# ethan-li-coding/AD-Census

Hardware: AMD Instinct MI355X
Metric: stereo pairs/s at 1920x1080 D=128 (ADCensusStereo::Match, images and disparity map resident in HBM) (higher is better)
Workload: dtype f32; 1 GPU; noise 1920x1080 D=128 (BASELINE.json configs[3]); batch=160 distinct pairs (seeds 12345+i), 668 per GPU (cycled), queue=static round-robin partition, in_flight_per_gpu=1, parallelism=replicas x1 (independent pairs), full=False

## Files before the change

### adcensus_amd/csrc/adc_internal.h

```cpp
#pragma once
#include <hip/hip_runtime.h>
#include <stdint.h>
#include <stddef.h>

#include "../../include/adcensus_c_api.h"

#define ADC_WAVE 64

#if !defined(ADC_VOL_NT) || ADC_VOL_NT
#define ADC_VOL_NT_STR " nt"
#define ADC_VOL_STORE(PTR, VAL) __builtin_nontemporal_store((VAL), (PTR))
#else
#define ADC_VOL_NT_STR ""
#define ADC_VOL_STORE(PTR, VAL) (*(PTR) = (VAL))
#endif


#ifdef ADC_FAULT_INJECTION
extern "C" int adc_test_fault_now(void);
#define ADC_HIP(call) (adc_test_fault_now() ? hipErrorOutOfMemory : (call))
#else
#define ADC_HIP(call) (call)
#endif

// ... 47 lines not shown
    int set;
    adc_raw_format fmt;
    uint32_t* rec;
    float *mx, *my;
    uint8_t* valid;
    uint8_t* raw;
    size_t raw_cap;
};

#define ADC_PIN_ARM 64
#define ADC_PIN_MEDIAN 0
#define ADC_PIN_CLOUD 8
#define ADC_PIN_SPECKLE 9
struct adc_handle {
    AdcParams p;
    int device;
    hipStream_t stream;
    hipStream_t heavy;
    hipEvent_t ev_in, ev_heavy_done;
    bool own_stream;

    uint8_t *img_l, *img_r;
    uint8_t *img_l_own, *img_r_own;
    uint8_t *gray_l, *gray_r;
    uint64_t *census_l, *census_r;
    uint8_t* arms;
    uint16_t *sup_h, *sup_v;
    int* armmax;
    uint32_t *rec_h, *rec_v;
    uint32_t *rec2_h, *rec2_v;
    float* agg_sink;
    uint8_t *cdiff_lh, *cdiff_lv, *cdiff_rh, *cdiff_rv;
    uint8_t* so_cls;
    float* so_seam;
    int so_seg_off;
    int so_nseg_last;
    int so_seam_redos;
    float *vol_a, *vol_b;
    float* lut_ad;
    float* lut_census;
    double* ray_sincos;
    float so_P1[3], so_P2[3];
    float *disp_l, *disp_r, *disp_tmp;
    uint8_t* label;
    uint8_t* elig;
    uint8_t* irv_bbox;
    int32_t* vote_list;
    int32_t* vote_evals_arr;
    int32_t* interp_list;
    int32_t* interp_counters;
    int32_t* ray_tab;
    int ray_tab_rows;
    int32_t* ray_lin;
    int itp_pitch, itp_ms;
    uint32_t* cost_rrec;
    uint32_t* cost_lrec;
    int rrec_pitch, rrec_padl;
    int armmax_host[2];
    int armmax_valid;
    int arm_known;
    int arm_redos;
    int agg_dual;
    int agg_dual_last;
    int agg_last_plan;
    int agg_switches;
    int agg_dual_runs;
    int armmax_small[2];
    int agg_gate, agg_gate_thr;
    int redo_partial;
    int match_pending;
    int fuse_cost;
    int agg_first_fused;
    int fuse_wta;
    int fuse_agg_so;
    int so_agg_fused;
    int agg_so_fusions;
    int32_t* pin_nz;
    long long rec_nz_host[2];
    int rec_nz_known;
    int in_redo;
    int agg_sparse_last;
    int agg_sparse_launches;
    int agg_gather_launches;
    int wta_left_done;
    float* med_hand;
    int med_hpitch;
    float* med_sink;
    int med_spec_off;
    int med_spec_last;
    int med_seg_last;
    int med_seg_off;
    int med_spec_fails;
    int force_median_fallback;
    int median_fallbacks;
    int32_t* pin_flags;
    int bgrx_valid;
    uint32_t* bgrx_l;
    uint16_t* st16;
    int st16_pitch;
    float* disp_vote;
    int irv_xcd_mode;
    int irv_grid;
    int irv_budget;
    int irv_used_hist[8];
    unsigned irv_used_pos;
    int irv_chain;
    int irv_pending;
    int irv_overflows;
    float *tail_disp_l, *tail_disp_tmp;
    void* irv_cold;
    unsigned char irv_cold_host[64];
    int irv_cold_valid, irv_cold_flip;
    int32_t* vote_counters;
    uint32_t* irv_px;
    uint8_t* chg_a;
    int chg_pitch;
    uint8_t* edge;
    uint8_t* itp_cells;
    uint8_t* pin_in;
    float* pin_out;
    AdcMatchReq req;
    AdcMapBuf map_buf[ADC_REQ_MAPS];
    uint32_t* out_words;
    void* os_cloud;
    uint32_t os_cloud_cap;
    int32_t sp_max_size;
    float sp_max_diff;
    int32_t* sp_parent;
    float* sp_map;
    AdcRectSide rect[2];
    uint8_t* pin_raw;
    size_t pin_raw_cap;
    int ev_set;
    int ev_has_right, ev_has_mask;
    float ev_occ_thres;
    int ev_cus;
    float* ev_g[2];
    uint8_t* ev_occ;
    uint8_t* ev_raw;
    size_t ev_raw_cap;
    uint64_t* ev_rep;
    uint64_t* ev_pin;
    int ev_pending;
    adc_eval_report ev_echo;
    adc_eval_report ev_report;
    int ev_report_valid;
    float* evs_disp;
    uint8_t* evs_prov;
    float* evs_conf;
    float* evs_err;
    uint8_t* evs_cls;
    int profiling, verbose;
    hipEvent_t ev[ADC_STAGE_COUNT + 1];
    hipEvent_t ev_agg[9];
    float stage_ms[ADC_STAGE_COUNT];
    float agg_pass_ms;
    int agg_launches;
    int agg_passes;
    const char* agg_kernel;
    uint32_t paper;
    uint8_t* arms_r;
    uint32_t* bgrx_r;
    int* armmax_r;
    float* vol_c;
    bool timings_pending;
    int64_t vote_rounds, vote_evals;
};

hipError_t adc_launch_gray_census(adc_handle* h);
hipError_t adc_launch_cost(adc_handle* h, float* vol_out);
hipError_t adc_launch_cost_records(adc_handle* h);
int adc_agg_small_L(const adc_handle* h);
double adc_agg_sparse_density(void);
double adc_agg_gather_density(void);
hipError_t adc_launch_arms(adc_handle* h);
hipError_t adc_launch_arms_left(adc_handle* h);
hipError_t adc_launch_sup_counts(adc_handle* h);
hipError_t adc_launch_arms_rest(adc_handle* h);
hipError_t adc_launch_aggregate_tail(adc_handle* h);
hipError_t adc_launch_records(adc_handle* h);
hipError_t adc_launch_aggregate(adc_handle* h, int iterations);
hipError_t adc_launch_so_classes(adc_handle* h, hipStream_t stream);
size_t adc_so_cls_bytes(int W, int H);
hipError_t adc_launch_scanline(adc_handle* h, int passes);
int adc_so_segments(const adc_handle* h, int* warm_out);
bool adc_so_can_fuse_agg(const adc_handle* h);
size_t adc_so_seam_bytes(int W, int H, int Dp);
hipError_t adc_launch_wta(adc_handle* h);
hipError_t adc_launch_wta_left(adc_handle* h);
hipError_t adc_paper_aggregate(adc_handle* h, int iterations);
hipError_t adc_paper_accumulate(adc_handle* h, float* acc, const float* src, int first, int last);
hipError_t adc_launch_lrcheck(adc_handle* h);
hipError_t adc_launch_confidence(adc_handle* h);
hipError_t adc_launch_provenance(adc_handle* h);
size_t adc_outputs_scratch_bytes(int W, int H);
hipError_t adc_launch_out_measure(adc_handle* h, const float* disp, const uint8_t* img);
hipError_t adc_launch_out_scan(adc_handle* h);
hipError_t adc_launch_out_emit(adc_handle* h, const float* disp, const uint8_t* img);
hipError_t adc_launch_disp16(adc_handle* h, const float* disp, float scale, uint16_t* out);
size_t adc_speckle_scratch_words(int W, int H);
hipError_t adc_launch_speckle_runs(adc_handle* h, const float* src, float max_diff);
hipError_t adc_launch_speckle_merge(adc_handle* h, const float* src, float max_diff);
hipError_t adc_launch_speckle_flatten(adc_handle* h, int32_t* labels);
hipError_t adc_launch_speckle_apply(adc_handle* h, const float* src, float* dst, uint8_t* prov, int max_size);
hipError_t adc_launch_rect_model_maps(adc_handle* h, int side, const adc_camera_model* m);
hipError_t adc_launch_rect_pack(adc_handle* h, int side);
hipError_t adc_launch_rect_remap(adc_handle* h, int side, const uint8_t* raw, uint8_t* bgr_out);
hipError_t adc_launch_rect_convert(adc_handle* h, int side, const uint8_t* raw, uint8_t* bgr_out);
static inline int adc_pix_code(int format) { return format & 0xff; }
static inline bool adc_pix_is16(int format) { const int c = format & 0xff; return c == ADC_PIX_GRAY16 || (c >= ADC_PIX_BAYER_RGGB16 && c <= ADC_PIX_BAYER_BGGR16); }
static inline int adc_pix_shift(int format) { const int b = (format >> 8) & 0xff; return adc_pix_is16(format) ? (b ? b : 16) - 8 : 0; }
size_t adc_eval_report_words(void);
hipError_t adc_launch_eval_gt(adc_handle* h, int side, int format, int pitch, float scale);
hipError_t adc_launch_eval_occ(adc_handle* h, int mode, float occ_thres);
hipError_t adc_launch_eval_measure(adc_handle* h, const float* disp, const uint8_t* prov, const float* conf, const float* thresholds, float* err, uint8_t* cls);
size_t adc_itp_cell_bytes(int W, int H, int ms);
#define ADC_MEDB_MAX_SEG 12
size_t adc_median_hand_rows(int H);
int adc_irv_probe_xcd_mode(int device);
int adc_irv_grid(size_t pixels);
size_t adc_irv_waves(int grid);
size_t adc_irv_px_words(int W, int H);
size_t adc_irv_list_entries(int W, int H, int D, int grid);
hipError_t adc_run_region_voting(adc_handle* h);
hipError_t adc_voting_finish(adc_handle* h, int* continued);
hipError_t adc_launch_interpolation(adc_handle* h);
hipError_t adc_launch_discontinuity(adc_handle* h);
hipError_t adc_launch_median(adc_handle* h);
hipError_t adc_median_fallback(adc_handle* h);
hipError_t adc_launch_pad_volume(adc_handle* h, const float* src_HWD, float* dst_HWDp);
hipError_t adc_launch_unpad_volume(adc_handle* h, const float* src_HWDp, float* dst_HWD);
```

### adcensus_amd/csrc/capi.hip

```cpp
#include "adc_internal.h"
#include "adc_device_fn.h"

#include <math.h>
#include <stdio.h>
#include <stdlib.h>
#include <string.h>
#include <string>
#include <vector>
#include <new>
#include <mutex>
#include <atomic>

static thread_local std::string g_last_error;

#ifdef ADC_FAULT_INJECTION
static std::atomic<long> g_fi_calls{0};
static std::atomic<long> g_fi_fail_at{[] { const char* e = getenv("ADC_TEST_FAIL_AT"); return e ? atol(e) : 0L; }()};
extern "C" int adc_test_fault_now(void) { const long n = ++g_fi_calls; return n == g_fi_fail_at.load(); }
extern "C" void adc_test_fail_at(long n) { g_fi_calls = 0; g_fi_fail_at = n; }
extern "C" long adc_test_hip_calls(void) { return g_fi_calls.load(); }
#endif

struct HostRange { const char* base; size_t bytes; };
static std::mutex g_host_mu;
// ... 1709 lines not shown
            if (e == hipSuccess && h->pin_nz) e = hipMemcpyAsync(h->pin_nz, h->armmax + ADC_NZ_BASE, 2 * ADC_NZ_SHARDS * ADC_NZ_STRIDE * sizeof(int32_t), hipMemcpyDeviceToHost, h->heavy);
            if (e == hipSuccess && h->pin_nz) e = hipStreamSynchronize(h->heavy);
            if (e == hipSuccess && h->pin_nz) {
                for (int c = 0; c < 2; c++) {
                    h->rec_nz_host[c] = 0;
                    for (int s = 0; s < ADC_NZ_SHARDS; s++) h->rec_nz_host[c] += h->pin_nz[(c * ADC_NZ_SHARDS + s) * ADC_NZ_STRIDE];
                }
                h->rec_nz_known = 1;
            }
            arg -= 200;
        }
        if (e == hipSuccess && arg >= 100) {
            if (h->paper & ADC_PAPER_RIGHT_ARMS) e = adc_launch_cost(h, h->vol_a);
            else { e = adc_launch_cost_records(h); h->fuse_cost = 1; }
            arg -= 100;
        }
        if (e == hipSuccess) e = adc_launch_aggregate(h, arg > 0 ? arg : 4);
        h->fuse_cost = 0;
        h->armmax_valid = 0;
        break;
    case ADC_RUN_SCANLINE:
        h->fuse_wta = arg >= 100 ? 1 : 0;
        h->wta_left_done = 0;
        e = adc_launch_scanline(h, arg >= 100 ? arg - 100 : arg);
        h->fuse_wta = 0;
        break;
    case ADC_RUN_WTA: e = adc_launch_wta(h); break;
    case ADC_RUN_LRCHECK: e = adc_launch_lrcheck(h); break;
    case ADC_RUN_REGION_VOTING:
        if (arg < 0) { h->irv_budget = -arg; return 0; }
        if (arg > 0) h->irv_budget = arg;
        e = adc_launch_sup_counts(h);
        if (e == hipSuccess) e = adc_run_region_voting(h);
        if (e == hipSuccess) e = hipStreamSynchronize(h->stream);
        if (e == hipSuccess) { int cont = 0; e = adc_voting_finish(h, &cont); }
        break;
    case ADC_RUN_INTERPOLATION: e = adc_launch_interpolation(h); break;
    case ADC_RUN_DISCONTINUITY: e = adc_launch_discontinuity(h); break;
    case ADC_RUN_MEDIAN:
        if (arg == 100) { h->force_median_fallback = 1; return 0; }
        if (arg == 101) { h->force_median_fallback = 2; return 0; }
        e = adc_launch_median(h);
        break;
    default: return 1;
    }
    if (e != hipSuccess) { set_error("adc_debug_run launch", e); return 2; }
    e = hipStreamSynchronize(h->heavy);
    if (e == hipSuccess) e = hipStreamSynchronize(h->stream);
    if (e != hipSuccess) { set_error("adc_debug_run sync", e); return 2; }
    if (stage == ADC_RUN_SCANLINE && h->so_nseg_last > 1) {
        int fails = 0;
        if (hipMemcpy(&fails, h->armmax + 2, sizeof(int), hipMemcpyDeviceToHost) != hipSuccess) { set_error("adc_debug_run: seam flag", hipGetLastError()); return 2; }
        if (fails != 0) {
            h->so_seg_off = 64;
            g_last_error = "adc_debug_run(ADC_RUN_SCANLINE): a speculative row segment failed its seam check; rerun with ADC_SO_SEG=1";
            return 3;
        }
    }
    if (stage == ADC_RUN_MEDIAN && h->pin_flags && h->pin_flags[ADC_PIN_MEDIAN] != 0) {
        e = adc_median_fallback(h);
        h->pin_flags[ADC_PIN_MEDIAN] = 0;
        h->median_fallbacks++;
        if (e != hipSuccess) { set_error("adc_debug_run: median fallback", e); return 2; }
    }
    return 0;
}

int64_t adc_debug_counter(adc_handle* h, int which)
{
    if (!h) return -1;
    switch (which) {
    case 0: return h->median_fallbacks;
    case 1: return h->irv_overflows;
    case 2: return h->arm_redos;
    case 9: return h->agg_switches;
    case 10: return h->agg_dual_runs;
    case 11: return h->redo_partial;
    case 12: return h->agg_dual;
    case 13: return h->agg_so_fusions;
    case 16: return h->agg_sparse_launches;
    case 17: return (int64_t)(adc_agg_sparse_density() * 1e6 + 0.5);
    case 20: return h->agg_gather_launches;
    case 21: return (int64_t)(adc_agg_gather_density() * 1e6 + 0.5);
    case 18: return h->rec_nz_known ? h->rec_nz_host[0] : -1;
    case 19: return h->rec_nz_known ? h->rec_nz_host[1] : -1;
    case 14: return h->irv_xcd_mode;
    case 15: return h->med_seg_last;
    case 3: return h->irv_budget;
    case 7: return h->med_spec_fails;
    case 8: return h->med_spec_last;
    case 4: return h->so_seam_redos;
    case 5: return h->so_nseg_last;
    case 6: {
        int v = -1;
        return hipMemcpy(&v, h->armmax + 2, sizeof(int), hipMemcpyDeviceToHost) == hipSuccess ? v : -1;
    }
    default: return -1;
    }
}

int adc_debug_voting_stats(adc_handle* h, int64_t* rounds, int64_t* evaluations)
{
    if (!h) return 1;
    if (rounds) *rounds = h->vote_rounds;
    if (evaluations) *evaluations = h->vote_evals;
    return 0;
}

}
```

### adcensus_amd/csrc/k_aggregate.hip

```cpp
#include "adc_internal.h"
#include "adc_device_fn.h"
#include <mutex>
#include "k_aggregate_rr.h"
#include "k_aggregate_rr2.h"
#include "k_agg_gather.h"

#define AGG_PF 8
#ifndef ADC_K4_TAILLOOP
#define ADC_K4_TAILLOOP 0
#endif
#ifndef ADC_K4_DIAG
#define ADC_K4_DIAG 0
#endif

__device__ __forceinline__ float agg_run(float acc, const float* q, int cnt)
{
    while (cnt >= 8) {
        const float t0 = q[0], t1 = q[64], t2 = q[128], t3 = q[192], t4 = q[256], t5 = q[320], t6 = q[384], t7 = q[448];
        acc += t0; acc += t1; acc += t2; acc += t3; acc += t4; acc += t5; acc += t6; acc += t7;
        q += 512;
        cnt -= 8;
    }
    switch (cnt) {
    case 7: { const float t0 = q[0], t1 = q[64], t2 = q[128], t3 = q[192], t4 = q[256], t5 = q[320], t6 = q[384];
// ... 566 lines not shown

int adc_agg_small_L(const adc_handle* h)
{
    static const int small_L_env = env_int("ADC_AGG_SMALL_L", 8);
    const int L = adc_imax(0, adc_imin(h->p.opt.cross_L1, 255));
    return adc_imin(small_L_env, L);
}

static int pick_nseg(long long nlines, int N, int L, int slots)
{
    int best = 1;
    long long best_cost = -1;
    for (int ns = 1; ns <= 16; ns++) {
        const int seg = (N + ns - 1) / ns;
        if (ns > 1 && seg < 2 * L) break;
        const long long rounds = (nlines * ns + slots - 1) / slots;
        const long long cost = rounds * (seg + (ns > 1 ? 2 * L : 0));
        if (best_cost < 0 || cost < best_cost) { best_cost = cost; best = ns; }
    }
    return best;
}

static int pick_chunk(long long nlines, int N, int L, int slots)
{
    const long long total = nlines * N;
    long long best_cost = -1;
    int best = N;
    auto consider = [&](long long c) {
        if (c < 1) c = 1;
        if (c < N && c < 4 * (long long)L) return;
        if (c > total) c = total;
        const long long waves = (total + c - 1) / c;
        const long long rounds = (waves + slots - 1) / slots;
        const bool aligned = c >= N ? (c % N == 0) : (N % c == 0);
        const long long pieces = aligned ? (c >= N ? c / N : 1) : (c >= N ? c / N + 2 : 2);
        const long long halo = (c < N || !aligned) ? 2LL * L : 0;
        const long long cost = rounds * (c + halo + 60 * pieces);
        if (best_cost < 0 || cost < best_cost) { best_cost = cost; best = (int)c; }
    };
    for (int k = 1; k <= 16; k++) consider((N + k - 1) / k);
    for (int k = 1; k <= 3; k++) consider((total + (long long)slots * k - 1) / ((long long)slots * k));
    return best;
}

static int agg_assumed_depth(const adc_handle* h, bool vert)
{
    const int assume_margin = env_int("ADC_AGG_ASSUME_MARGIN", 1);
    const int Lknown = adc_imax(1, h->armmax_host[vert ? 1 : 0]) + (h->armmax_valid == 2 ? assume_margin : 0);
    return adc_imin(adc_agg_small_L(h), Lknown);
}

static bool agg_small_vpl2(const adc_handle* h, bool pair)
{
    static const int vpl2_env = env_int("ADC_AGG_VPL2", 1);
    return (vpl2_env == 1 || (vpl2_env == 2 && pair)) && h->p.Dp % 128 == 0;
}

#define AGG_SPARSE_MAX_DENSITY 0.105
double adc_agg_sparse_density(void)
{
    const char* e = getenv("ADC_AGG_SPARSE_DENSITY");
    return e ? atof(e) : AGG_SPARSE_MAX_DENSITY;
}
static bool agg_sparse_wanted(const adc_handle* h, bool vert, bool pair)
{
    const char* e = getenv("ADC_AGG_SPARSE");
    if (e && atoi(e) == 0) return false;
    if (h->agg_gate || h->in_redo || !(h->armmax_valid == 1 || h->armmax_valid == 2) || !h->rec_nz_known) return false;
    if (!agg_small_vpl2(h, pair)) return false;
    return (double)h->rec_nz_host[vert ? 1 : 0] <= adc_agg_sparse_density() * (double)h->p.W * (double)h->p.H;
}

#define AGG_GATHER_MAX_DENSITY AGG_SPARSE_MAX_DENSITY
double adc_agg_gather_density(void)
{
    const char* e = getenv("ADC_AGG_GATHER_DENSITY");
    return e ? atof(e) : AGG_GATHER_MAX_DENSITY;
}
static bool agg_gather_wanted(const adc_handle* h, bool vert)
{
    const char* e = getenv("ADC_AGG_GATHER");
    if (e && atoi(e) == 0) return false;
    return (double)h->rec_nz_host[vert ? 1 : 0] <= adc_agg_gather_density() * (double)h->p.W * (double)h->p.H;
}

template <bool VERT, bool DIVIDE, bool COSTIN = false, bool PAIR = false>
static hipError_t launch_pass(adc_handle* h, const float* src, float* dst, int which = 0, bool sparse = false)
{
    const bool gather = sparse && agg_gather_wanted(h, VERT);
    const AdcParams& p = h->p;
    const int L = adc_imax(0, adc_imin(p.opt.cross_L1, 255));
    const int N = VERT ? p.H : p.W;
    const int small_L = adc_agg_small_L(h);
    if (sparse && (COSTIN || which != 1 || !agg_small_vpl2(h, PAIR))) return hipErrorInvalidValue;
    for (int variant = 0; variant < 2; variant++) {
        if (variant == 1 && (small_L <= 0 || small_L >= L)) break;
        if ((which == 1 && variant == 0 && small_L > 0 && small_L < L) || (which == 2 && variant == 1)) continue;
        const int Lv = variant ? ((which == 1 && h->armmax_valid) ? agg_assumed_depth(h, VERT) : small_L) : L;
        static const bool regring_env = env_int("ADC_AGG_REGRING", 1) != 0;
        const bool regring = variant == 0 && regring_env && Lv >= 1 && 2 * Lv + 1 <= AGG_RING_REGS;
        static const bool rr2_env = env_int("ADC_AGG_RR2", 1) != 0;
        const bool rr2 = regring && rr2_env && !PAIR && p.Dp % 128 == 0 && 2 * Lv + 1 <= RR2_SLOTS;
        const int vpl = rr2 ? 2 : ((variant == 1 && !COSTIN && agg_small_vpl2(h, PAIR)) ? 2 : 1);
        const long long nlines = (long long)(VERT ? p.W : p.H) * (p.Dp / (64 * vpl));
        const size_t ring_bytes = regring ? 0 : (size_t)(2 * Lv + 1) * 64 * sizeof(float) * vpl;
        const size_t ldsv = ring_bytes + (COSTIN ? (768 + 64) * sizeof(float) : 0) + ((PAIR && !regring) ? ring_bytes + (2 * Lv + 1) * 4 + 64 : 0);
        const int waves_per_cu = regring ? ((PAIR || rr2) ? 8 : 16) : adc_imax(1, adc_imin(32, (int)((160 * 1024) / ((ldsv + 511) / 512 * 512))));
        int nseg = env_int(VERT ? "ADC_AGG_VSEG" : "ADC_AGG_HSEG", 0);
        if (nseg < 1) nseg = pick_nseg(nlines, N, PAIR ? 2 * Lv : Lv, 256 * waves_per_cu);
        int seg_len = (N + nseg - 1) / nseg;
        if (seg_len < 1) seg_len = 1;
        nseg = (N + seg_len - 1) / seg_len;
        const long long waves = nlines * nseg;
        const int per_xcd = (int)((waves + 7) / 8);
        const bool both = which == 0 && small_L > 0 && small_L < L;
        const bool verify = variant == 1 && which == 1 && h->armmax_valid == 2;
        int sv = both ? variant : (verify ? 2 : -1), sl = both ? small_L : (verify ? Lv : 0x7fffffff);
        if (h->agg_gate) { sv = h->agg_gate; sl = h->agg_gate_thr; }
        AggCostIn ci;
        ci.rrec = reinterpret_cast<const uint4*>(h->cost_rrec);
        ci.lrec = reinterpret_cast<const uint4*>(h->cost_lrec);
        ci.lut_ad = h->lut_ad;
        ci.lut_census = h->lut_census;
        ci.rpitch = h->rrec_pitch; ci.padl = h->rrec_padl; ci.dmin = p.dmin; ci.D = p.D;
        if (!COSTIN)
            h->agg_kernel = rr2 ? "k_agg_rr2 (register ring of VGPR pairs, 2 disparities per lane, one pass per launch)"
                          : regring ? (PAIR ? "k_agg_regring_pair (two register rings, dividing pass + next first pass per launch)"
                                            : "k_agg_regring (register ring, 1 disparity per lane, one pass per launch)")
                          : (variant && gather) ? (PAIR ? "k_agg_gather<.., PAIR> + k_agg_apply (SPARSE launch, gather form: dividing pass + next first pass, only changed pixels computed)"
                                                        : "k_agg_gather + k_agg_apply (SPARSE launch, gather form: one pass per launch, only changed pixels computed)")
                          : (variant && sparse) ? (PAIR ? "k_agg_march<.., PAIR, SPARSE> + k_agg_apply (LDS small rings: dividing pass + next first pass per launch, only changed pixels stored)"
                                                        : "k_agg_march<.., SMALL, SPARSE> + k_agg_apply (LDS small ring, one pass per launch, only changed pixels stored)")
                          : variant ? (PAIR ? "k_agg_march<.., PAIR> (LDS small rings: dividing pass + next first pass per launch)"
                                            : "k_agg_march<.., SMALL> (LDS small ring, one pass per launch)")
                                    : "k_agg_march (LDS full ring, one pass per launch)";
        if (rr2) {
            int chunk_len = env_int(VERT ? "ADC_AGG_VCHUNK" : "ADC_AGG_HCHUNK", 0);
            if (chunk_len < 1) chunk_len = pick_chunk(nlines, N, Lv, 256 * waves_per_cu);
            const long long total = nlines * N;
            const int nwaves = (int)((total + chunk_len - 1) / chunk_len);
            const int pxc = (nwaves + 7) / 8;
            if constexpr (COSTIN)
                hipLaunchKernelGGL(k_agg_rr2_cost, dim3((unsigned)pxc * 8), dim3(64), ldsv, h->heavy, dst,
                                   reinterpret_cast<const uint2*>(h->rec2_h), p.W, p.H, p.Dp, Lv, chunk_len, nwaves, pxc, h->armmax, sv, sl, ci);
            else if constexpr (!PAIR)
                hipLaunchKernelGGL((k_agg_rr2<VERT, DIVIDE>), dim3((unsigned)pxc * 8), dim3(64), 0, h->heavy, src, dst,
                                   reinterpret_cast<const uint2*>(VERT ? h->rec2_v : h->rec2_h), p.W, p.H, p.Dp, Lv, chunk_len, nwaves,
                                   pxc, h->armmax, sv, sl);
        } else if (regring) {
            if constexpr (COSTIN)
                hipLaunchKernelGGL(k_agg_regring_cost, dim3((unsigned)per_xcd * 8), dim3(64), ldsv, h->heavy, src, dst,
                                   VERT ? h->rec_v : h->rec_h, p.W, p.H, p.Dp, Lv, seg_len, nseg, per_xcd, h->armmax, sv, sl, ci);
            else if constexpr (PAIR)
                hipLaunchKernelGGL((k_agg_regring_pair<VERT>), dim3((unsigned)per_xcd * 8), dim3(64), 0, h->heavy, src, dst,
                                   reinterpret_cast<const uint2*>(VERT ? h->rec2_v : h->rec2_h), p.W, p.H, p.Dp, Lv, seg_len, nseg,
                                   per_xcd, h->armmax, sv, sl, h->agg_sink);
            else
                hipLaunchKernelGGL((k_agg_regring<VERT, DIVIDE>), dim3((unsigned)per_xcd * 8), dim3(64), 0, h->heavy, src, dst,
                                   reinterpret_cast<const uint2*>(VERT ? h->rec2_v : h->rec2_h), p.W, p.H, p.Dp, Lv, seg_len, nseg,
                                   per_xcd, h->armmax, sv, sl, h->agg_sink);
        } else if (variant && vpl == 2) {
            if constexpr (!COSTIN) {
                if (sparse) {
                    const long long P = (long long)p.W * p.H;
                    if (gather) {
                        hipLaunchKernelGGL((k_agg_gather<VERT, DIVIDE, PAIR>), dim3((unsigned)((P + 255) / 256)), dim3(256), 0, h->heavy, src, dst,
                                           VERT ? h->rec_v : h->rec_h, p.W, p.H, p.Dp, h->armmax, sv, sl);
                        h->agg_gather_launches++;
                    } else
                        hipLaunchKernelGGL((k_agg_march<VERT, DIVIDE, true, false, PAIR, 2, true>), dim3((unsigned)per_xcd * 8), dim3(64), ldsv, h->heavy, src, dst,
                                           VERT ? h->rec_v : h->rec_h, p.W, p.H, p.Dp, Lv, seg_len, nseg, per_xcd, h->armmax, sv, sl, ci);
                    hipLaunchKernelGGL((k_agg_apply<VERT>), dim3((unsigned)((P + 255) / 256)), dim3(256), 0, h->heavy, dst, const_cast<float*>(src),
                                       VERT ? h->rec_v : h->rec_h, p.W, p.H, p.Dp, (DIVIDE || PAIR) ? 1 : 0, h->armmax, sv, sl);
                    h->agg_sparse_launches++;
                    h->agg_sparse_last = 1;
                } else
                    hipLaunchKernelGGL((k_agg_march<VERT, DIVIDE, true, false, PAIR, 2>), dim3((unsigned)per_xcd * 8), dim3(64), ldsv, h->heavy, src, dst,
                                       VERT ? h->rec_v : h->rec_h, p.W, p.H, p.Dp, Lv, seg_len, nseg, per_xcd, h->armmax, sv, sl, ci);
            }
        } else if (variant)
            hipLaunchKernelGGL((k_agg_march<VERT, DIVIDE, true, COSTIN, PAIR>), dim3((unsigned)per_xcd * 8), dim3(64), ldsv, h->heavy, src, dst,
                               VERT ? h->rec_v : h->rec_h, p.W, p.H, p.Dp, Lv, seg_len, nseg, per_xcd, h->armmax, sv, sl, ci);
        else
            hipLaunchKernelGGL((k_agg_march<VERT, DIVIDE, false, COSTIN, PAIR>), dim3((unsigned)per_xcd * 8), dim3(64), ldsv, h->heavy, src, dst,
                               VERT ? h->rec_v : h->rec_h, p.W, p.H, p.Dp, Lv, seg_len, nseg, per_xcd, h->armmax, sv, sl, ci);
    }
    return hipGetLastError();
}

struct AggSeq { int launches, passes; float* result; bool first_fused; };
static hipError_t agg_sequence(adc_handle* h, int iterations, bool dry, bool first_into_cur, bool marks, AggSeq* out)
{
    static const bool pair_env = env_int("ADC_AGG_PAIR", 1) != 0;
    static const int pair_full = env_int("ADC_AGG_PAIR_FULL", 0);
    static const bool regring_on = env_int("ADC_AGG_REGRING", 1) != 0;
    hipError_t e = hipSuccess;
    const int Lfull = adc_imax(0, adc_imin(h->p.opt.cross_L1, 255));
    const bool regring_fits = regring_on && Lfull >= 1 && 2 * Lfull + 1 <= AGG_RING_REGS;
    const bool lds_fits = (size_t)(2 * Lfull + 1) * 64 * sizeof(float) + (768 + 64) * sizeof(float) <= 150 * 1024;
    const bool marching = true;
    const bool prof = marks && !dry && h->profiling;
    const int small_L = adc_agg_small_L(h);
    const bool small_ok = small_L > 0 && small_L < Lfull;
    int which_h = 0, which_v = 0;
    if (h->armmax_valid == 3 && marching) {
        which_h = which_v = 2;
    } else if (h->armmax_valid && marching) {
        which_h = (small_ok && h->armmax_host[0] <= small_L) ? 1 : 2;
        which_v = (small_ok && h->armmax_host[1] <= small_L) ? 1 : 2;
    }
    float* cur = h->vol_a;
    float* oth = h->vol_b;
    bool horizontal_first = true;
    int launch = 0;
    int passes = 0;
    bool second_done = false;
    bool first_fused = false;
    for (int k = 0; k < iterations && e == hipSuccess; k++) {
        const bool hf = horizontal_first;
        if (!second_done) {
            if (prof && launch < 2) hipEventRecord(h->ev_agg[launch], h->heavy);
            bool swap = true;
            if (hf) {
                const bool fused = k == 0 && h->fuse_cost && lds_fits;
                if (k == 0) first_fused = fused;
                if (fused) {
                    swap = !first_into_cur;
                    if (!dry) e = launch_pass<false, false, true>(h, cur, swap ? oth : cur, which_h);
                } else {
                    const bool sp = which_h == 1 && agg_sparse_wanted(h, false, false);
                    if (!dry) e = launch_pass<false, false>(h, cur, oth, which_h, sp);
                    swap = !sp;
                }
            } else {
                const bool sp = which_v == 1 && agg_sparse_wanted(h, true, false);
                if (!dry) e = launch_pass<true, false>(h, cur, oth, which_v, sp);
                swap = !sp;
            }
            if (swap) { float* t = cur; cur = oth; oth = t; }
            launch++;
            passes++;
        }
        second_done = false;
        if (e != hipSuccess) break;
        if (prof && launch < 2) hipEventRecord(h->ev_agg[launch], h->heavy);
        const int wsec = hf ? which_v : which_h;
        if (!hf && k + 1 == iterations && iterations == 4 && h->fuse_agg_so && !h->agg_gate && marching && which_h == 1 &&
            (h->armmax_valid == 1 || h->armmax_valid == 2) && agg_assumed_depth(h, false) <= 4 && adc_so_can_fuse_agg(h)) {
            if (!dry) { h->so_agg_fused = 1; h->agg_so_fusions++; }
            break;
        }
        const bool pair = pair_env && marching && k + 1 < iterations &&
                          (wsec == 1 || (wsec == 2 && (pair_full >= 2 || (pair_full == 1 && regring_fits))));
        const bool sparse = wsec == 1 && agg_sparse_wanted(h, hf, pair);
        if (!dry) {
            if (hf) {
                if (pair) e = launch_pass<true, true, false, true>(h, cur, oth, wsec, sparse);
                else e = launch_pass<true, true>(h, cur, oth, which_v, sparse);
            } else {
                if (pair) e = launch_pass<false, true, false, true>(h, cur, oth, wsec, sparse);
                else e = launch_pass<false, true>(h, cur, oth, which_h, sparse);
            }
// ... 91 lines not shown
```

### adcensus_amd/csrc/k_cost.hip

```cpp
#include "adc_internal.h"
#include "adc_device_fn.h"

#define CT_W 32
#define CT_H 8
#define CT_LW (CT_W + 6)
#define CT_LH (CT_H + 8)

__global__ __launch_bounds__(CT_W* CT_H) void k_gray_census(const uint8_t* __restrict__ img_l,
                                                             const uint8_t* __restrict__ img_r,
                                                             uint8_t* __restrict__ gray_l, uint8_t* __restrict__ gray_r,
                                                             uint64_t* __restrict__ census_l,
                                                             uint64_t* __restrict__ census_r, int W, int H, int census5)
{
    __shared__ uint8_t tile[CT_LH][CT_LW + 2];
    const uint8_t* img = blockIdx.z == 0 ? img_l : img_r;
    uint8_t* gray = blockIdx.z == 0 ? gray_l : gray_r;
    uint64_t* census = blockIdx.z == 0 ? census_l : census_r;
    const int x0 = blockIdx.x * CT_W, y0 = blockIdx.y * CT_H;
    const int tid = threadIdx.y * CT_W + threadIdx.x;
    for (int i = tid; i < CT_LH * CT_LW; i += CT_W * CT_H) {
        const int ly = i / CT_LW, lx = i % CT_LW;
        const int gx = x0 + lx - 3, gy = y0 + ly - 4;
        uint8_t g = 0;
        if (gx >= 0 && gx < W && gy >= 0 && gy < H) {
            const uint8_t* p = img + ((size_t)gy * W + gx) * 3;
            g = adc_gray(p[0], p[1], p[2]);
        }
        tile[ly][lx] = g;
    }
    __syncthreads();
    const int x = x0 + threadIdx.x, y = y0 + threadIdx.y;
    if (x >= W || y >= H) return;
    const int lx = threadIdx.x + 3, ly = threadIdx.y + 4;
    const uint8_t c = tile[ly][lx];
    gray[(size_t)y * W + x] = c;
    uint64_t v = 0;
    if (census5) {
        if (W > 5 && H > 5 && y >= 2 && y < H - 2 && x >= 2 && x < W - 2) {
#pragma unroll
            for (int r = -2; r <= 2; r++)
#pragma unroll
                for (int cc = -2; cc <= 2; cc++) {
                    v <<= 1;
                    v += (tile[ly + r][lx + cc] < c) ? 1u : 0u;
                }
        }
    } else if (W > 9 && H > 7 && y >= 4 && y < H - 4 && x >= 3 && x < W - 3) {
#pragma unroll
        for (int r = -4; r <= 4; r++)
#pragma unroll
            for (int cc = -3; cc <= 3; cc++) {
                v <<= 1;
                v += (tile[ly + r][lx + cc] < c) ? 1u : 0u;
            }
    }
    census[(size_t)y * W + x] = v;
}

hipError_t adc_launch_gray_census(adc_handle* h)
{
    const AdcParams& p = h->p;
    dim3 grid((p.W + CT_W - 1) / CT_W, (p.H + CT_H - 1) / CT_H, 2), block(CT_W, CT_H, 1);
    hipLaunchKernelGGL(k_gray_census, grid, block, 0, h->heavy, h->img_l, h->img_r, h->gray_l, h->gray_r, h->census_l,
                       h->census_r, p.W, p.H, (h->paper & ADC_PAPER_CENSUS5X5) ? 1 : 0);
    return hipGetLastError();
}

#define COST_TX 32
#define COST_MAXSEG (COST_TX + ADC_MAX_DISP_RANGE)

template <int VPL>
__global__ __launch_bounds__(256) void k_cost(const uint8_t* __restrict__ img_l, const uint8_t* __restrict__ img_r,
                                              const uint64_t* __restrict__ census_l,
                                              const uint64_t* __restrict__ census_r, const float* __restrict__ lut_ad,
                                              const float* __restrict__ lut_census, float* __restrict__ vol, int W,
                                              int H, int dmin, int D)
{
    constexpr int Dp = 64 * VPL;
    __shared__ float sA[768];
    __shared__ float sC[64];
    __shared__ uint32_t sBgr[COST_MAXSEG];
    __shared__ uint64_t sCen[COST_MAXSEG];

    const int y = blockIdx.y;
// ... 25 lines not shown
        const int bl = pl[0], gl = pl[1], rl = pl[2];
        const uint64_t cl = census_l[(size_t)y * W + x];
        float out[VPL];
#pragma unroll
        for (int k = 0; k < VPL; k++) {
            const int di = lane * VPL + k;
            float c = 0.0f;
            if (di < D) {
                const int xr = x - (di + dmin);
                const uint32_t pr = sBgr[xr - xr_lo];
                if (pr == 0xFFFFFFFFu) {
                    c = 1.0f;
                } else {
                    const int ad = adc_iabs(bl - (int)(pr & 255u)) + adc_iabs(gl - (int)((pr >> 8) & 255u)) +
                                   adc_iabs(rl - (int)((pr >> 16) & 255u));
                    const int hm = __popcll(cl ^ sCen[xr - xr_lo]);
                    c = sA[ad] - sC[hm];
                }
            }
            out[k] = c;
        }
        float* dst = vol + ((size_t)y * W + x) * Dp + lane * VPL;
        if constexpr (VPL == 1) dst[0] = out[0];
        else if constexpr (VPL == 2) *reinterpret_cast<float2*>(dst) = make_float2(out[0], out[1]);
        else {
#pragma unroll
            for (int q = 0; q < VPL; q += 4) *reinterpret_cast<float4*>(dst + q) = make_float4(out[q], out[q + 1], out[q + 2], out[q + 3]);
        }
    }
}

hipError_t adc_launch_cost(adc_handle* h, float* vol_out)
{
    const AdcParams& p = h->p;
    dim3 grid((p.W + COST_TX - 1) / COST_TX, p.H, 1), block(256, 1, 1);
#define LAUNCH(V)                                                                                                     \
    hipLaunchKernelGGL(k_cost<V>, grid, block, 0, h->heavy, h->img_l, h->img_r, h->census_l, h->census_r, h->lut_ad, \
                       h->lut_census, vol_out, p.W, p.H, p.dmin, p.D)
    if (p.VPL == 1) LAUNCH(1);
    else if (p.VPL == 2) LAUNCH(2);
    else if (p.VPL == 4) LAUNCH(4);
    else if (p.VPL == 8) LAUNCH(8);
    else if (p.VPL == 16) LAUNCH(16);
    else LAUNCH(32);
#undef LAUNCH
    return hipGetLastError();
}

__global__ __launch_bounds__(256) void k_cost_records(const uint8_t* __restrict__ img_l, const uint8_t* __restrict__ img_r,
                                                      const uint64_t* __restrict__ census_l,
                                                      const uint64_t* __restrict__ census_r, uint4* __restrict__ lrec,
                                                      uint4* __restrict__ rrec, int W, int H, int pitch, int padl)
{
    const int y = blockIdx.y;
    const int i = blockIdx.x * 256 + threadIdx.x;
    if (i < pitch) {
        const int c = i - padl;
        uint4 r = make_uint4(0xFFFFFFFFu, 0u, 0u, 0u);
        if (c >= 0 && c < W) {
            const size_t p = (size_t)y * W + c;
            const uint64_t cs = census_r[p];
            r = make_uint4((uint32_t)img_r[3 * p] | ((uint32_t)img_r[3 * p + 1] << 8) | ((uint32_t)img_r[3 * p + 2] << 16),
                           (uint32_t)cs, (uint32_t)(cs >> 32), 0u);
        }
        rrec[(size_t)y * pitch + i] = r;
    }
    if (i < W) {
        const size_t p = (size_t)y * W + i;
        const uint64_t cs = census_l[p];
        lrec[p] = make_uint4((uint32_t)img_l[3 * p] | ((uint32_t)img_l[3 * p + 1] << 8) | ((uint32_t)img_l[3 * p + 2] << 16),
                             (uint32_t)cs, (uint32_t)(cs >> 32), 0u);
    }
}

hipError_t adc_launch_cost_records(adc_handle* h)
{
    const AdcParams& p = h->p;
    hipLaunchKernelGGL(k_cost_records, dim3((h->rrec_pitch + 255) / 256, p.H), dim3(256), 0, h->heavy, h->img_l, h->img_r,
                       h->census_l, h->census_r, reinterpret_cast<uint4*>(h->cost_lrec), reinterpret_cast<uint4*>(h->cost_rrec),
                       p.W, p.H, h->rrec_pitch, h->rrec_padl);
    return hipGetLastError();
}

__global__ void k_pad_volume(const float* __restrict__ src, float* __restrict__ dst, size_t P, int D, int Dp, int to_padded)
{
    const size_t n = P * (size_t)Dp;
    for (size_t i = (size_t)blockIdx.x * blockDim.x + threadIdx.x; i < n; i += (size_t)gridDim.x * blockDim.x) {
        const size_t px = i / Dp;
        const int d = (int)(i % Dp);
        if (to_padded) dst[i] = d < D ? src[px * D + d] : 0.0f;
        else if (d < D) dst[px * D + d] = src[i];
    }
}

hipError_t adc_launch_pad_volume(adc_handle* h, const float* src_HWD, float* dst_HWDp)
{
    const AdcParams& p = h->p;
    hipLaunchKernelGGL(k_pad_volume, dim3(2048), dim3(256), 0, h->stream, src_HWD, dst_HWDp, (size_t)p.W * p.H, p.D, p.Dp, 1);
    return hipGetLastError();
}
hipError_t adc_launch_unpad_volume(adc_handle* h, const float* src_HWDp, float* dst_HWD)
{
    const AdcParams& p = h->p;
    hipLaunchKernelGGL(k_pad_volume, dim3(2048), dim3(256), 0, h->stream, src_HWDp, dst_HWD, (size_t)p.W * p.H, p.D, p.Dp, 0);
    return hipGetLastError();
}
```

### adcensus_amd/csrc/k_scanline.hip

```cpp
#include "adc_internal.h"
#include "adc_device_fn.h"

template <int CTRL>
__device__ __forceinline__ float dpp_mov(float old, float src)
{
    return __int_as_float(__builtin_amdgcn_update_dpp(__float_as_int(old), __float_as_int(src), CTRL, 0xf, 0xf, false));
}

template <bool DPP>
__device__ __forceinline__ float wave_min_f32(float v)
{
    if constexpr (DPP) {
        asm("s_nop 1\n\tv_min_f32_dpp %0, %0, %0 row_ror:1 row_mask:0xf bank_mask:0xf\n\t"
            "s_nop 1\n\tv_min_f32_dpp %0, %0, %0 row_ror:2 row_mask:0xf bank_mask:0xf\n\t"
            "s_nop 1\n\tv_min_f32_dpp %0, %0, %0 row_ror:4 row_mask:0xf bank_mask:0xf\n\t"
            "s_nop 1\n\tv_min_f32_dpp %0, %0, %0 row_ror:8 row_mask:0xf bank_mask:0xf\n\t"
            "s_nop 1\n\tv_min_f32_dpp %0, %0, %0 row_bcast:15 row_mask:0xa bank_mask:0xf\n\t"
            "s_nop 1\n\tv_min_f32_dpp %0, %0, %0 row_bcast:31 row_mask:0xc bank_mask:0xf\n\t"
            "s_nop 1"
            : "+v"(v));
        return __int_as_float(__builtin_amdgcn_readlane(__float_as_int(v), 63));
    } else {
#pragma unroll
        for (int m = 32; m >= 1; m >>= 1) {
// ... 157 lines not shown
{
    if constexpr (VPL == 1) return rmap[off];
    else if constexpr (VPL == 2) { uint16_t v; __builtin_memcpy(&v, rmap + off, 2); return v; }
    else { uint32_t v; __builtin_memcpy(&v, rmap + off, 4); return v; }
}
template <int VPL>
__device__ __forceinline__ void so_rmap_load_words(const uint8_t* __restrict__ rmap, int off, uint32_t* w)
{
    if constexpr (VPL <= 4) w[0] = so_rmap_load<VPL>(rmap, off);
    else {
#pragma unroll
        for (int q = 0; q < VPL / 4; q++) __builtin_memcpy(&w[q], rmap + off + 4 * q, 4);
    }
}

#ifndef SO_INTERIOR
#define SO_INTERIOR 1
#endif
#ifndef SO_FAST
#define SO_FAST 1
#endif
#define SO_V0 96
#define SO_RC(U) (SO_V0 + 2 * (U))
#define SO_RR(U) (SO_V0 + 32 + (U))
#define SO_RW(G) (SO_V0 + 48 + (G))
#define SO_CLOBBERS "v96", "v97", "v98", "v99", "v100", "v101", "v102", "v103", "v104", "v105", "v106", "v107", "v108", "v109", "v110", "v111", "v112", "v113", "v114", "v115", "v116", "v117", "v118", "v119", "v120", "v121", "v122", "v123", "v124", "v125", "v126", "v127", "v128", "v129", "v130", "v131", "v132", "v133", "v134", "v135", "v136", "v137", "v138", "v139", "v140", "v141", "v142", "v143", "v144", "v145", "v146", "v147"
#define SO_AGG_LA 4
template <int VPL, bool VERT, bool DPP, bool WTA, bool PIN, bool SEG = false, bool AGG = false>
__device__ __forceinline__ void so_body(const float* __restrict__ src, float* __restrict__ dst,
                                        const uint32_t* __restrict__ c1w, int ngr,
                                        const uint8_t* __restrict__ rmap, int W, int H, int D, int dmin, int tso,
                                        int dir, float P1a, float P1b, float P1c, float P2a, float P2b, float P2c,
                                        float* __restrict__ disp, int allow_fast, int nseg = 1, int warm = 0, float* __restrict__ seam = nullptr,
                                        const uint32_t* __restrict__ aggrec = nullptr)
{
    static_assert(!AGG || (SEG && !PIN && !VERT && !WTA && VPL == 2), "fused aggregation: the L->R row pass, two disparities per lane, compiler-allocated slots");
    static_assert(!WTA || DPP, "the fused winner-takes-all relies on the uniform (SGPR) path minimum of the DPP reduction");
    static_assert(!SEG || (!WTA && !VERT && VPL <= 2), "verified segments: row passes of the asm-prefetch kernels");
    constexpr int Dp = 64 * VPL;
    __shared__ float2 so_tab[4];
    if (threadIdx.x < 4) {
        const int c = threadIdx.x;
        so_tab[c] = make_float2(c == 0 ? P1a : (c == 1 ? P1b : P1c), c == 0 ? P2a : (c == 1 ? P2b : P2c));
    }
    __syncthreads();
    const int wave = __builtin_amdgcn_readfirstlane(threadIdx.x >> 6);
    const int lane = threadIdx.x & 63;
    const int npaths = VERT ? W : H;
    SoGeom g;
    g.W = W; g.H = H; g.dir = dir; g.lane = lane;
    g.path = __builtin_amdgcn_readfirstlane((int)blockIdx.x * (int)(blockDim.x >> 6) + wave);
    int seg = 0;
    if constexpr (SEG) {
        seg = g.path / npaths;
        g.path -= seg * npaths;
        if (seg >= nseg) return;
    }
    if (g.path >= npaths) return;
    g.plen = VERT ? H : W;
    int e0 = 0, e1 = g.plen, efirst = 0;
    if constexpr (SEG) {
        e1 = adc_so_seg_start(g.plen, nseg, warm, seg + 1);
        if (seg > 0) {
            efirst = adc_so_seg_start(g.plen, nseg, warm, seg);
            e0 = efirst - warm - 1;
        }
    }
    const int plen_v = e1 - e0;
    g.d0 = lane * VPL;
    const uint32_t* c1p = c1w + (size_t)g.path * ngr;
    const int cl_last = g.d0 + VPL - 1 + dmin;

    float agr[AGG ? 2 * SO_AGG_LA + 1 : 1][VPL];
    const uint32_t* recp = AGG ? aggrec + (size_t)g.path * W : nullptr;
#define SO_AGG_PUSH(C)                                                                                         \
    do {                                                                                                       \
        _Pragma("unroll") for (int t_ = 2 * SO_AGG_LA; t_ > 0; t_--)                                           \
            _Pragma("unroll") for (int k_ = 0; k_ < VPL; k_++) agr[t_][k_] = agr[t_ - 1][k_];                  \
        _Pragma("unroll") for (int k_ = 0; k_ < VPL; k_++) agr[0][k_] = (C)[k_];                               \
    } while (0)
#define SO_AGG_EVAL(EIDX, C)                                                                                   \
    do {                                                                                                       \
        const uint32_t rec_ = recp[(EIDX)];                                                                    \
        const int top_ = SO_AGG_LA + (int)(rec_ & 255u), bot_ = SO_AGG_LA - (int)((rec_ >> 8) & 255u);         \
        const float cnt_ = (float)(rec_ >> 16);                                                                \
        _Pragma("unroll") for (int k_ = 0; k_ < VPL; k_++) {                                                   \
            float acc_ = 0.0f;                                                                                 \
            _Pragma("unroll") for (int t_ = 2 * SO_AGG_LA; t_ >= 0; t_--) acc_ += (t_ <= top_ && t_ >= bot_) ? agr[t_][k_] : 0.0f; \
            (C)[k_] = acc_ / cnt_;                                   \
        }                                                                                                      \
    } while (0)
    float Lp[VPL];
    float minLp;
    {
        const size_t pix = so_pixel<VERT>(g, e0);
        float c[VPL];
        if constexpr (AGG) {
#pragma unroll
            for (int t_ = 0; t_ <= 2 * SO_AGG_LA; t_++) {
                const int er_ = adc_imax(0, adc_imin(g.plen - 1, e0 + SO_AGG_LA - t_));
                vload<VPL>(src + so_pixel<VERT>(g, er_) * Dp + g.d0, agr[t_]);
            }
            SO_AGG_EVAL(e0, c);
        } else
        vload<VPL>(src + pix * Dp + g.d0, c);
        if (!SEG || seg == 0) vstore<VPL>(dst + pix * Dp + g.d0, c);
        float lmin = ADC_LARGE_FLOAT;
#pragma unroll
        for (int k = 0; k < VPL; k++) {
            Lp[k] = (g.d0 + k) < D ? c[k] : ADC_LARGE_FLOAT;
            lmin = Lp[k] < lmin ? Lp[k] : lmin;
        }
        minLp = wave_min_f32<DPP>(lmin);
    }
    float upN = lane_up<DPP>(Lp[VPL - 1], ADC_LARGE_FLOAT, lane);
    float dnN = lane_down<DPP>(Lp[0], ADC_LARGE_FLOAT, lane);
    int wtaB = 0;
    float wtaC1 = 0.f, wtaC2 = 0.f, wtaM = 0.f;
#define SO_WTA(I)                                                                                          \
    if constexpr (WTA) {                                                                                   \
        int bi_ = 0x7fffffff;                                                                              \
        _Pragma("unroll") for (int k = 0; k < VPL; k++)                                                    \
        {                                                                                                  \
            const unsigned long long m_ = __ballot(Lp[k] == minLp);                                        \
            const int c_ = m_ ? (int)__builtin_ctzll(m_) * VPL + k : 0x7fffffff;                           \
            bi_ = c_ < bi_ ? c_ : bi_;                                                                     \
        }                                                                                                  \
         \
        const int best_ = minLp < ADC_LARGE_FLOAT ? bi_ + dmin : 0;                                        \
         \
        const int idx_ = (best_ - dmin) & (64 * VPL - 1);                                                  \
        const int kw_ = idx_ % VPL, lw_ = idx_ / VPL;                                                      \
        float s1_ = upN, s2_ = VPL == 1 ? dnN : Lp[VPL == 1 ? 0 : 1];                                      \
        _Pragma("unroll") for (int k = 1; k < VPL; k++)                                                    \
        {                                                                                                  \
            s1_ = kw_ == k ? Lp[k - 1] : s1_;                                                              \
            s2_ = kw_ == k ? (k == VPL - 1 ? dnN : Lp[k == VPL - 1 ? k : k + 1]) : s2_;                    \
        }                                                                                                  \
        const int c1_ = __builtin_amdgcn_readlane(__float_as_int(s1_), lw_);                               \
        const int c2_ = __builtin_amdgcn_readlane(__float_as_int(s2_), lw_);                               \
        const int slot_ = (I)&63;                                                                          \
        const bool mine_ = lane == slot_;                        \
        wtaB = mine_ ? best_ : wtaB;                                                                       \
        wtaC1 = mine_ ? __int_as_float(c1_) : wtaC1;                                                       \
        wtaC2 = mine_ ? __int_as_float(c2_) : wtaC2;                                                       \
        wtaM = mine_ ? minLp : wtaM;                                                                       \
        if (slot_ == 63 || (I) == g.plen - 1) {                                                            \
            const int e_ = ((I) & ~63) + lane;                       \
            if (e_ <= (I)) {                                                                               \
                float o_;                                                                                  \
                if (wtaB == dmin || wtaB == dmin + D - 1) o_ = ADC_INVALID_FLOAT;                          \
                else if (wtaB - 1 - dmin < 0 || wtaB + 1 - dmin >= D) o_ = (float)wtaB;                    \
                else o_ = adc_subpixel(wtaB, wtaC1, wtaC2, wtaM);                                          \
                disp[so_pixel<VERT>(g, e_)] = o_;                                                          \
            }                                                                                              \
        }                                                                                                  \
    }
    SO_WTA(0);
    if (plen_v <= 1) return;

    int mcur = dir > 0 ? e0 + 1 : g.plen - 2 - e0;
    const int dpad = (D + VPL - 1) / VPL * VPL;
#define SO_STEP(I, E)                                                                                      \
    do {                                                                                                   \
        const int x_ = VERT ? g.path : mcur;    \
        int off_[VPL];                                                                                     \
        if (SO_INTERIOR && adc_so_interior(x_, W, dmin, dpad))  \
            adc_so_class_offsets_interior<VPL>((E).rb, (E).c1, tso, off_);                                 \
        else                                                                                               \
            adc_so_class_offsets<VPL>((E).rb, (E).c1, x_ - cl_last, W, tso, W >= 3 && x_ - dmin >= 1, off_);   \
        const float up_ = upN;                                           \
        const float dn_ = dnN;                                          \
// ... 561 lines not shown
```

Baseline: 311.5 pairs/s.

## Fuse cost computation into first horizontal aggregation pass for sparse-record inputs

Adds a kernel that computes AD-Census matching costs from left/right pixel records on the fly and sums them over each pixel's horizontal arm. It replaces the first cost-input horizontal aggregation pass when the record density is low, so the cost volume is never read back. It also adds a fast path in the scanline fused-aggregation macro that copies the centre value when a record leaves the pixel unchanged. The cost is extra recomputation per arm element and LDS use, and the fused path is gated by density and LDS-fit checks.

```diff
diff --git a/adcensus_amd/csrc/adc_internal.h b/adcensus_amd/csrc/adc_internal.h
--- a/adcensus_amd/csrc/adc_internal.h
+++ b/adcensus_amd/csrc/adc_internal.h
@@ -153,6 +153,7 @@
     int agg_sparse_last;
     int agg_sparse_launches;
     int agg_gather_launches;
+    int agg_flat_launches;
     int wta_left_done;
     float* med_hand;
     int med_hpitch;
@@ -241,9 +242,12 @@
 hipError_t adc_launch_gray_census(adc_handle* h);
 hipError_t adc_launch_cost(adc_handle* h, float* vol_out);
 hipError_t adc_launch_cost_records(adc_handle* h);
+bool adc_cost_agg_flat_fits(const adc_handle* h, int cap);
+hipError_t adc_launch_cost_agg_flat(adc_handle* h, float* dst, int cap, int small_variant, int small_L);
 int adc_agg_small_L(const adc_handle* h);
 double adc_agg_sparse_density(void);
 double adc_agg_gather_density(void);
+double adc_cost_flat_density(void);
 hipError_t adc_launch_arms(adc_handle* h);
 hipError_t adc_launch_arms_left(adc_handle* h);
 hipError_t adc_launch_sup_counts(adc_handle* h);
diff --git a/adcensus_amd/csrc/capi.hip b/adcensus_amd/csrc/capi.hip
--- a/adcensus_amd/csrc/capi.hip
+++ b/adcensus_amd/csrc/capi.hip
@@ -1815,6 +1815,13 @@
     case 17: return (int64_t)(adc_agg_sparse_density() * 1e6 + 0.5);
     case 20: return h->agg_gather_launches;
     case 21: return (int64_t)(adc_agg_gather_density() * 1e6 + 0.5);
+    case 22: return h->agg_flat_launches;
+    case 23: return (int64_t)(adc_cost_flat_density() * 1e6 + 0.5);
+    case 24: {
+        float ms = 0.f;
+        if (!h->profiling || h->agg_dual_last || h->agg_launches < 1 || hipEventElapsedTime(&ms, h->ev_agg[0], h->ev_agg[1]) != hipSuccess) return -1;
+        return (int64_t)((double)ms * 1e6 + 0.5);
+    }
     case 18: return h->rec_nz_known ? h->rec_nz_host[0] : -1;
     case 19: return h->rec_nz_known ? h->rec_nz_host[1] : -1;
     case 14: return h->irv_xcd_mode;
diff --git a/adcensus_amd/csrc/k_aggregate.hip b/adcensus_amd/csrc/k_aggregate.hip
--- a/adcensus_amd/csrc/k_aggregate.hip
+++ b/adcensus_amd/csrc/k_aggregate.hip
@@ -672,6 +672,20 @@
     const char* e = getenv("ADC_AGG_GATHER");
     if (e && atoi(e) == 0) return false;
     return (double)h->rec_nz_host[vert ? 1 : 0] <= adc_agg_gather_density() * (double)h->p.W * (double)h->p.H;
+}
+
+#define COST_FLAT_MAX_DENSITY AGG_SPARSE_MAX_DENSITY
+double adc_cost_flat_density(void)
+{
+    const char* e = getenv("ADC_COST_FLAT_DENSITY");
+    return e ? atof(e) : COST_FLAT_MAX_DENSITY;
+}
+static bool cost_flat_wanted(const adc_handle* h, int which, int cap)
+{
+    const char* e = getenv("ADC_COST_FLAT");
+    if (e && atoi(e) == 0) return false;
+    if (which != 1 || !agg_sparse_wanted(h, false, false) || !adc_cost_agg_flat_fits(h, cap)) return false;
+    return (double)h->rec_nz_host[0] <= adc_cost_flat_density() * (double)h->p.W * (double)h->p.H;
 }
 
 template <bool VERT, bool DIVIDE, bool COSTIN = false, bool PAIR = false>
@@ -768,6 +782,10 @@
                     hipLaunchKernelGGL((k_agg_march<VERT, DIVIDE, true, false, PAIR, 2>), dim3((unsigned)per_xcd * 8), dim3(64), ldsv, h->heavy, src, dst,
                                        VERT ? h->rec_v : h->rec_h, p.W, p.H, p.Dp, Lv, seg_len, nseg, per_xcd, h->armmax, sv, sl, ci);
             }
+        } else if (variant && COSTIN && cost_flat_wanted(h, which, Lv)) {
+            const hipError_t ef = adc_launch_cost_agg_flat(h, dst, Lv, sv, sl);
+            if (ef != hipSuccess) return ef;
+            h->agg_flat_launches++;
         } else if (variant)
             hipLaunchKernelGGL((k_agg_march<VERT, DIVIDE, true, COSTIN, PAIR>), dim3((unsigned)per_xcd * 8), dim3(64), ldsv, h->heavy, src, dst,
                                VERT ? h->rec_v : h->rec_h, p.W, p.H, p.Dp, Lv, seg_len, nseg, per_xcd, h->armmax, sv, sl, ci);
diff --git a/adcensus_amd/csrc/k_cost.hip b/adcensus_amd/csrc/k_cost.hip
--- a/adcensus_amd/csrc/k_cost.hip
+++ b/adcensus_amd/csrc/k_cost.hip
@@ -1,5 +1,8 @@
 #include "adc_internal.h"
 #include "adc_device_fn.h"
+#include "k_aggregate_rr.h"
+#include "k_aggregate_rr2.h"
+#include "k_cost_flat.h"
 
 #define CT_W 32
 #define CT_H 8
@@ -191,6 +194,121 @@
     return hipGetLastError();
 }
 
+#define CF_PW 32
+#define CF_HALO 16
+#define CF_TX (4 * CF_PW)
+#define CF_LDS_MAX (48 * 1024)
+typedef float cf_f2 __attribute__((ext_vector_type(2)));
+
+template <bool PAD>
+__global__ __launch_bounds__(256) void k_cost_agg_flat(float* __restrict__ dst, const uint32_t* __restrict__ rec, int W, int H, int Dp,
+                                                       int cap, int tiles, const int* __restrict__ armmax, int small_variant,
+                                                       int small_L, AggCostIn ci)
+{
+    if (agg_gate_skip(armmax, small_variant, small_L, false)) return;
+    extern __shared__ __attribute__((aligned(16))) uint32_t cf_lds[];
+    const int n = CF_TX + Dp - 1 + 2 * cap;
+    float* lutA = reinterpret_cast<float*>(cf_lds);
+    float* lutC = lutA + 768;
+    uint32_t* sB = cf_lds + 768 + 64;
+    uint32_t* sC0 = sB + n;
+    uint32_t* sC1 = sC0 + n;
+    const int tid = threadIdx.x;
+    const int y = (int)blockIdx.x / tiles;
+    const int x0 = ((int)blockIdx.x - y * tiles) * CF_TX;
+    for (int i = tid; i < 766; i += 256) lutA[i] = ci.lut_ad[i];
+    if (tid < 64) lutC[tid] = ci.lut_census[tid];
+    const int col_lo = x0 - cap - ci.dmin - (Dp - 1);
+    const uint4* rrow = ci.rrec + (size_t)y * ci.rpitch;
+    for (int i = tid; i < n; i += 256) {
+        int gi = ci.padl + col_lo + i;
+        gi = gi < 0 ? 0 : (gi >= ci.rpitch ? ci.rpitch - 1 : gi);
+        const uint4 r = rrow[gi];
+        sB[i] = r.x;
+        sC0[i] = r.y;
+        sC1[i] = r.z;
+    }
+    __syncthreads();
+
+    const int wave = __builtin_amdgcn_readfirstlane(tid >> 6), lane = tid & 63;
+    const int xw = x0 + wave * CF_PW;
+    if (xw >= W) return;
+    const int xl = adc_imax(0, adc_imin(W - 1, xw - CF_HALO + lane));
+    const uint4 lr = ci.lrec[(size_t)y * W + xl];
+    const uint32_t myrec = rec[(size_t)y * W + xl];
+    const int npx = adc_imin(CF_PW, W - xw);
+    const uint32_t* qB = sB + (xw - x0) + cap + (Dp - 1) - 2 * lane;
+    const uint32_t* qC0 = qB + n;
+    const uint32_t* qC1 = qC0 + n;
+    float* pd = dst + ((size_t)y * W + xw) * Dp + 2 * lane;
+    for (int p = 0; p < npx; p++, qB++, qC0++, qC1++, pd += Dp) {
+        const int li = CF_HALO + p;
+        const uint32_t rq = (uint32_t)__builtin_amdgcn_readlane((int)myrec, li);
+        auto left_at = [&](int t) -> CfRec {
+            CfRec l;
+            if (li + t >= 0 && li + t < 64) {
+                l.b = (uint32_t)__builtin_amdgcn_readlane((int)lr.x, li + t);
+                l.c0 = (uint32_t)__builtin_amdgcn_readlane((int)lr.y, li + t);
+                l.c1 = (uint32_t)__builtin_amdgcn_readlane((int)lr.z, li + t);
+            } else {
+                const uint4 q = ci.lrec[(size_t)y * W + xw + p + t];
+                l.b = (uint32_t)__builtin_amdgcn_readfirstlane((int)q.x);
+                l.c0 = (uint32_t)__builtin_amdgcn_readfirstlane((int)q.y);
+                l.c1 = (uint32_t)__builtin_amdgcn_readfirstlane((int)q.z);
+            }
+            return l;
+        };
+        int lo = 0, hi = 0;
+        const bool single = (rq & 0xFFFFu) == 0u;
+        if (!single) cost_flat_arms(rq, xw + p, W, cap, &lo, &hi);
+        for (int c = 0; c < Dp; c += 128) {
+            const bool pad[2] = {c + 2 * lane >= ci.D, c + 2 * lane + 1 >= ci.D};
+            auto right_at = [&](int t, int k) -> CfRec {
+                CfRec r;
+                r.b = qB[t - c - k];
+                r.c0 = qC0[t - c - k];
+                r.c1 = qC1[t - c - k];
+                return r;
+            };
+            float out[2];
+            if (single) cost_flat_span<2, PAD>(0, 0, left_at, right_at, lutA, lutC, pad, out);
+            else cost_flat_span<2, PAD>(lo, hi, left_at, right_at, lutA, lutC, pad, out);
+            cf_f2 v;
+            v.x = out[0];
+            v.y = out[1];
+            ADC_VOL_STORE(reinterpret_cast<cf_f2*>(pd + c), v);
+        }
+    }
+}
+
+static size_t cost_agg_flat_lds(const adc_handle* h, int cap)
+{
+    return (size_t)(768 + 64 + 3 * (CF_TX + h->p.Dp - 1 + 2 * cap)) * 4;
+}
+bool adc_cost_agg_flat_fits(const adc_handle* h, int cap)
+{
+    return h->p.Dp % 128 == 0 && cap >= 0 && cost_agg_flat_lds(h, cap) <= CF_LDS_MAX;
+}
+hipError_t adc_launch_cost_agg_flat(adc_handle* h, float* dst, int cap, int small_variant, int small_L)
+{
+    const AdcParams& p = h->p;
+    if (!adc_cost_agg_flat_fits(h, cap)) return hipErrorInvalidValue;
+    AggCostIn ci;
+    ci.rrec = reinterpret_cast<const uint4*>(h->cost_rrec);
+    ci.lrec = reinterpret_cast<const uint4*>(h->cost_lrec);
+    ci.lut_ad = h->lut_ad;
+    ci.lut_census = h->lut_census;
+    ci.rpitch = h->rrec_pitch; ci.padl = h->rrec_padl; ci.dmin = p.dmin; ci.D = p.D;
+    const int tiles = (p.W + CF_TX - 1) / CF_TX;
+    if (p.D == p.Dp)
+        hipLaunchKernelGGL(k_cost_agg_flat<false>, dim3((unsigned)tiles * p.H), dim3(256), cost_agg_flat_lds(h, cap), h->heavy, dst, h->rec_h,
+                           p.W, p.H, p.Dp, cap, tiles, h->armmax, small_variant, small_L, ci);
+    else
+        hipLaunchKernelGGL(k_cost_agg_flat<true>, dim3((unsigned)tiles * p.H), dim3(256), cost_agg_flat_lds(h, cap), h->heavy, dst, h->rec_h,
+                           p.W, p.H, p.Dp, cap, tiles, h->armmax, small_variant, small_L, ci);
+    return hipGetLastError();
+}
+
 __global__ void k_pad_volume(const float* __restrict__ src, float* __restrict__ dst, size_t P, int D, int Dp, int to_padded)
 {
     const size_t n = P * (size_t)Dp;
diff --git a/adcensus_amd/csrc/k_cost_flat.h b/adcensus_amd/csrc/k_cost_flat.h
--- /dev/null
+++ b/adcensus_amd/csrc/k_cost_flat.h
@@ -0,0 +1,60 @@
+#pragma once
+
+#ifndef RR_EMUL
+#define CF_FN __device__ __forceinline__
+#define CF_SAD_U8(A, B) __builtin_amdgcn_sad_u8((A), (B), 0u)
+#define CF_POPC(X) ((uint32_t)__popc(X))
+#else
+#include <cstdint>
+#define CF_FN static inline
+static inline uint32_t cf_sad_u8(uint32_t a, uint32_t b)
+{
+    uint32_t s = 0;
+    for (int k = 0; k < 4; k++) {
+        const int x = (int)((a >> (8 * k)) & 255u), y = (int)((b >> (8 * k)) & 255u);
+        s += (uint32_t)(x > y ? x - y : y - x);
+    }
+    return s;
+}
+#define CF_SAD_U8(A, B) cf_sad_u8((A), (B))
+#define CF_POPC(X) ((uint32_t)__builtin_popcount(X))
+#endif
+
+#define CF_MARKER 0xFFFFFFFFu
+
+struct CfRec { uint32_t b, c0, c1; };
+
+CF_FN float cost_flat_term(const CfRec& r, const CfRec& l, const float* lutA, const float* lutC, bool pad)
+{
+    const uint32_t ad = CF_SAD_U8(r.b, l.b);
+    const uint32_t hm = CF_POPC(r.c0 ^ l.c0) + CF_POPC(r.c1 ^ l.c1);
+    float cv = lutA[ad < 766u ? ad : 765u] - lutC[hm & 63u];
+    cv = r.b == CF_MARKER ? 1.0f : cv;
+    return pad ? 0.0f : cv;
+}
+
+CF_FN void cost_flat_arms(uint32_t rec, int x, int W, int cap, int* lo, int* hi)
+{
+    const int a = (int)(rec & 255u), b = (int)((rec >> 8) & 255u);
+    const int la = a < x ? a : x, hb = b < W - 1 - x ? b : W - 1 - x;
+    *lo = la < cap ? la : cap;
+    *hi = hb < cap ? hb : cap;
+}
+
+template <int NV, bool PAD, class LeftAt, class RightAt>
+CF_FN void cost_flat_span(int lo, int hi, LeftAt left_at, RightAt right_at, const float* lutA, const float* lutC, const bool* pad,
+                          float* out)
+{
+    if (lo == 0 && hi == 0) {
+        const CfRec l = left_at(0);
+        for (int k = 0; k < NV; k++) out[k] = cost_flat_term(right_at(0, k), l, lutA, lutC, PAD && pad[k]);
+        return;
+    }
+    float acc[NV];
+    for (int k = 0; k < NV; k++) acc[k] = 0.0f;
+    for (int t = -lo; t <= hi; t++) {
+        const CfRec l = left_at(t);
+        for (int k = 0; k < NV; k++) acc[k] = acc[k] + cost_flat_term(right_at(t, k), l, lutA, lutC, PAD && pad[k]);
+    }
+    for (int k = 0; k < NV; k++) out[k] = acc[k];
+}
diff --git a/adcensus_amd/csrc/k_scanline.hip b/adcensus_amd/csrc/k_scanline.hip
--- a/adcensus_amd/csrc/k_scanline.hip
+++ b/adcensus_amd/csrc/k_scanline.hip
@@ -263,12 +263,20 @@
 #define SO_AGG_EVAL(EIDX, C)                                                                                   \
     do {                                                                                                       \
         const uint32_t rec_ = recp[(EIDX)];                                                                    \
-        const int top_ = SO_AGG_LA + (int)(rec_ & 255u), bot_ = SO_AGG_LA - (int)((rec_ >> 8) & 255u);         \
-        const float cnt_ = (float)(rec_ >> 16);                                                                \
-        _Pragma("unroll") for (int k_ = 0; k_ < VPL; k_++) {                                                   \
-            float acc_ = 0.0f;                                                                                 \
-            _Pragma("unroll") for (int t_ = 2 * SO_AGG_LA; t_ >= 0; t_--) acc_ += (t_ <= top_ && t_ >= bot_) ? agr[t_][k_] : 0.0f; \
-            (C)[k_] = acc_ / cnt_;                                   \
+         \
+         \
+         \
+         \
+        if (!adc_rec_changes_pixel(rec_, true)) {                                                              \
+            _Pragma("unroll") for (int k_ = 0; k_ < VPL; k_++) (C)[k_] = agr[SO_AGG_LA][k_];                   \
+        } else {                                                                                               \
+            const int top_ = SO_AGG_LA + (int)(rec_ & 255u), bot_ = SO_AGG_LA - (int)((rec_ >> 8) & 255u);     \
+            const float cnt_ = (float)(rec_ >> 16);                                                            \
+            _Pragma("unroll") for (int k_ = 0; k_ < VPL; k_++) {                                               \
+                float acc_ = 0.0f;                                                                             \
+                _Pragma("unroll") for (int t_ = 2 * SO_AGG_LA; t_ >= 0; t_--) acc_ += (t_ <= top_ && t_ >= bot_) ? agr[t_][k_] : 0.0f; \
+                (C)[k_] = acc_ / cnt_;                               \
+            }                                                                                                  \
         }                                                                                                      \
     } while (0)
     float Lp[VPL];
```

Measured after the change: 327.1 pairs/s, median of 6. +5.0%, better.
